# turnDeep/Computational-Chemistry-AI

Measured on AMD Instinct MI355X. Metric: scf_iterations_per_sec, higher is better.
Workload: dtype f64

## Files before the change

computational-chemistry-ai_amd/csrc/mi355scf.hip:

```cpp

#include <hip/hip_runtime.h>
#include <algorithm>
#include <chrono>
#include <cmath>
#include <cstdarg>
#include <cstdint>
#include <cstdio>
#include <cstring>
#include <numeric>
#include <string>
#include <thread>
#include <mutex>
#include <map>
#include <unordered_map>
#include <vector>

#include "../../include/mi355scf.h"
#include "rys_tables.h"

#define LMAX 4
#define LMAX_1E 3
#define NPC ((LMAX + 1) * (LMAX + 2) / 2)
#define BLK 8
#define ATM_SLOTS 6
// ... 329 lines not shown
    double opt_tpq_maxprim = 32.0;
    int opt_eri_tpq = 1;
    int opt_jk_multi_batch = 8;
    int opt_jk_pair = -1;
    int opt_tri_tiles = 1;
    int tri = 1;
    int opt_jk_cache_mb = 160;
    int opt_grad_rows = 1;
    int opt_grad_rows_min = 20;
    int opt_grad_live = 1;
    int opt_jk_kjlt = 0;
    int opt_jk_dpp = 1;
    int opt_jk_pipe = -1;
    int opt_ao_order = 1;
    int opt_ket_cluster = 1;
    int opt_xf_mlds = 0;
    int opt_rys_qpw_maxcomp = 256;
    double opt_rys_qpw_maxprim = 4.0;
    int opt_xf_qpw_max = 40;
    int opt_work_mb = 2048;
    int opt_grad_work_mb = 1024;
    int opt_vmat_fold_mt = 3;
    int opt_rys_fine = 1;
    int opt_eri_fused = 0;
    int opt_task_table = 1;
    int opt_prim_lds = 0;
    int opt_xcd_map = 1;
    int ao_order = 0;
    int *d_perm = nullptr, *d_iperm = nullptr;
    std::vector<int> perm, iperm;
    int opt_vmat_xcd = 1;
    int opt_vmat_wgs = 0;
    int opt_sp2_direct = 0;
    double *d_xt_scratch = nullptr;
};

static inline int pc_index(int la, int lb) { return la * (la + 1) / 2 + lb; }
static inline int ne_of(int la, int lb) { int n = 0; for (int e = la; e <= la + lb; e++) n += ncart(e); return n; }

static double gaussian_int(int n, double a) { return std::tgamma((n + 1) * 0.5) / (2.0 * std::pow(a, (n + 1) * 0.5)); }

static int set_tile_order(mi_ctx *c, int order)
{
    if (c->ao_order == order) return 0;
    const int nbas = c->nbas;
    std::vector<int> seq(nbas);
    std::iota(seq.begin(), seq.end(), 0);
    if (order == 1) std::stable_sort(seq.begin(), seq.end(), [&](int a, int b) { return c->shells[a].l < c->shells[b].l; });
    c->perm.assign(std::max(c->nao, 1), 0);
    c->iperm.assign(std::max(c->nao, 1), 0);
    int pos = 0;
    for (int s_ : seq) {
        ShellH &S = c->shells[s_];
        S.ao = pos;
        for (int m = 0; m < 2 * S.l + 1; m++) { c->perm[S.ao_nat + m] = pos + m; c->iperm[pos + m] = S.ao_nat + m; }
        pos += 2 * S.l + 1;
    }
    HIPCHK(hipMemcpy(c->d_perm, c->perm.data(), sizeof(int) * c->perm.size(), hipMemcpyHostToDevice));
    HIPCHK(hipMemcpy(c->d_iperm, c->iperm.data(), sizeof(int) * c->iperm.size(), hipMemcpyHostToDevice));
    c->ao_order = order;
    return 0;
}

struct HostStash {
    std::mutex mu;
    std::vector<double> h_M, h_prim;
// ... 222 lines not shown
        std::lock_guard<std::mutex> g(H.mu);
        if (c->h_M.capacity() > H.h_M.capacity()) H.h_M.swap(c->h_M);
        if (c->h_prim.capacity() > H.h_prim.capacity()) H.h_prim.swap(c->h_prim);
        if (c->tiles.capacity() > H.tiles.capacity()) H.tiles.swap(c->tiles);
        if (c->tile_off.capacity() > H.tile_off.capacity()) H.tile_off.swap(c->tile_off);
    }
    delete c;
}

extern "C" int mi_ctx_nao(const mi_ctx *c) { return c ? c->nao : -1; }

extern "C" int mi_set_option(mi_ctx *c, const char *key, double value)
{
    if (!c || !key) return fail("mi_set_option: null argument");
    std::string k(key);
    if (k == "runmax") c->opt_runmax = (int)value;
    else if (k == "omega") {
        if (!(value >= 0.0) || !std::isfinite(value)) return fail("mi_set_option: omega must be finite and >= 0");
        c->opt_omega = value;
    }
    else if (k == "jk_waves") c->opt_jk_waves = (int)value;
    else if (k == "jk_nt") c->opt_jk_nt = (int)value;
    else if (k == "jk_pipe") c->opt_jk_pipe = (int)value;
    else if (k == "jk_dpp") c->opt_jk_dpp = (int)value;
    else if (k == "jk_kjlt") c->opt_jk_kjlt = (int)value;
    else if (k == "grad_live") c->opt_grad_live = (int)value;
    else if (k == "grad_rows") c->opt_grad_rows = (int)value;
    else if (k == "grad_rows_min") c->opt_grad_rows_min = (int)value;
    else if (k == "grad_rows_g32") g_rows_g32 = (int)value;
    else if (k == "jk_cache_mb") c->opt_jk_cache_mb = (int)value;
    else if (k == "jk_pair") c->opt_jk_pair = (int)value;
    else if (k == "jk_multi_batch") c->opt_jk_multi_batch = (int)value;
    else if (k == "sp2_direct") c->opt_sp2_direct = (int)value;
    else if (k == "vmat_wgs") c->opt_vmat_wgs = (int)value;
    else if (k == "vmat_xcd") c->opt_vmat_xcd = (int)value;
    else if (k == "tri_tiles") c->opt_tri_tiles = (int)value;
    else if (k == "ao_order") c->opt_ao_order = (int)value;
    else if (k == "ket_cluster") c->opt_ket_cluster = (int)value;
    else if (k == "xcd_map") c->opt_xcd_map = (int)value;
    else if (k == "prim_lds") c->opt_prim_lds = (int)value;
    else if (k == "task_table") c->opt_task_table = (int)value;
    else if (k == "eri_fused") c->opt_eri_fused = (int)value;
    else if (k == "rys_fine") c->opt_rys_fine = (int)value;
    else if (k == "vmat_fold_mt") c->opt_vmat_fold_mt = (int)value;
    else if (k == "work_mb") c->opt_work_mb = (int)value;
    else if (k == "grad_work_mb") c->opt_grad_work_mb = (int)value;
    else if (k == "rys_qpw_maxcomp") c->opt_rys_qpw_maxcomp = (int)value;
    else if (k == "rys_qpw_maxprim") c->opt_rys_qpw_maxprim = value;
    else if (k == "xf_qpw_max") c->opt_xf_qpw_max = (int)value;
    else if (k == "xf_mlds") c->opt_xf_mlds = (int)value;
    else if (k == "eri_tpq") c->opt_eri_tpq = (int)value;
    else if (k == "tpq_maxprim") c->opt_tpq_maxprim = value;
    else if (k == "xf_mfma_min") c->opt_xf_mfma_min = (int)value;
    else if (k == "grad_dtol") c->opt_grad_dtol = value;
    else if (k == "grad_prefetch") c->opt_grad_prefetch = (int)value;
    else return fail("mi_set_option: unknown key '%s'", key);
    return 0;
}

#define NC1 10

__device__ inline void cart_pow(int l, int idx, int &x, int &y, int &z)
{
    int n = 0;
    for (int lx = l; lx >= 0; lx--) {
        int cnt = l - lx + 1;
// ... 6439 lines not shown
    hipLaunchKernelGGL(finalize_fock_kernel, dim3((unsigned)((nn + 255) / 256)), dim3(256), 0, st, c->d_Jacc, with_k ? c->d_Kacc : nullptr,
                       c->ldp, d_h, d_Vun, d_D, kscale, c->nao, d_F, d_part, c->d_perm);
    HIPCHK(hipGetLastError());
    return 0;
}

__global__ __launch_bounds__(256) void commutator_norm_kernel(const double *M, int n, double *E, double *part)
{
    __shared__ double sh[4];
    size_t idx = (size_t)blockIdx.x * blockDim.x + threadIdx.x;
    double s = 0.0;
    if (idx < (size_t)n * n) {
        int r = (int)(idx / n), cidx = (int)(idx - (size_t)r * n);
        double v = M[idx] - M[(size_t)cidx * n + r];
        E[idx] = v;
        s = v * v;
    }
    for (int o = 32; o > 0; o >>= 1) s += __shfl_xor(s, o);
    if ((threadIdx.x & 63) == 0) sh[threadIdx.x >> 6] = s;
    __syncthreads();
    if (threadIdx.x == 0) part[blockIdx.x] = (sh[0] + sh[1]) + (sh[2] + sh[3]);
}

extern "C" int mi_commutator_norm(mi_ctx *c, const double *d_M, double *d_E, double *d_part, void *stream)
{
    if (!c || !d_M || !d_E || !d_part) return fail("mi_commutator_norm: null argument");
    int n = c->nao;
    hipLaunchKernelGGL(commutator_norm_kernel, dim3((unsigned)(((size_t)n * n + 255) / 256)), dim3(256), 0, (hipStream_t)stream, d_M, n, d_E,
                       d_part);
    HIPCHK(hipGetLastError());
    return 0;
}

#define VM_T 64
#define VM_KS 64
#define VM_PAD 2
__global__ __launch_bounds__(256) void xc_vmat_kernel(const double *__restrict__ A, const double *__restrict__ W, int nao, int64_t ng,
                                                      int64_t kchunk, double *C, int xcd_order)
{
    __shared__ double Pa[VM_T][VM_KS + VM_PAD], Pb[VM_T][VM_KS + VM_PAD];
    const int nt = (nao + VM_T - 1) / VM_T, ntt = nt * nt;
    const int L = (int)blockIdx.x;
    int tile, split;
    if (xcd_order) { split = (L & 7) + 8 * (L / (8 * ntt)); tile = (L >> 3) % ntt; }
    else { tile = L % ntt; split = L / ntt; }
    const int m0 = (tile / nt) * VM_T, n0 = (tile % nt) * VM_T;
    const int64_t kbeg = (int64_t)split * kchunk, kend = min(ng, kbeg + kchunk);
    const int wave = threadIdx.x >> 6, lane = threadIdx.x & 63;
    const int qm = (wave >> 1) * 32, qn = (wave & 1) * 32;
    const bool va0 = m0 + qm < nao, va1 = m0 + qm + 16 < nao, vb0 = n0 + qn < nao, vb1 = n0 + qn + 16 < nao;
    d4_t acc[2][2];
#pragma unroll
    for (int a = 0; a < 2; a++)
#pragma unroll
        for (int b = 0; b < 2; b++) acc[a][b] = d4_t{0.0, 0.0, 0.0, 0.0};
    constexpr int PER = VM_T * VM_KS / 256;
    double ra[PER], rb[PER];
    auto gload = [&](int64_t k0) {
#pragma unroll
        for (int u = 0; u < PER; u++) {
            int idx = u * 256 + threadIdx.x;
            int r = idx / VM_KS, k = idx - r * VM_KS;
            int64_t g = k0 + k;
            ra[u] = (m0 + r < nao && g < kend) ? A[(size_t)(m0 + r) * ng + g] : 0.0;
            rb[u] = (n0 + r < nao && g < kend) ? W[(size_t)(n0 + r) * ng + g] : 0.0;
        }
// ... 607 lines not shown
```

computational-chemistry-ai_amd/python/mi355scf/engine.py:

```python
import ctypes
import os

import numpy as np
import torch

_HERE = os.path.dirname(os.path.abspath(__file__))
_CSRC = os.path.normpath(os.path.join(_HERE, "..", "..", "csrc"))
LIB_PATH = os.path.join(_CSRC, "libmi355scf.so")
_lib = None


class EngineError(RuntimeError):
    pass


class EngineOutOfMemory(EngineError):

    def __init__(self, msg, need_bytes, free_bytes):
        super().__init__(msg)
        self.need_bytes, self.free_bytes = need_bytes, free_bytes


MI_ERR_NOMEM = -2

# ... 58 lines not shown
        L.mi_xc_aow.argtypes = [vp, vp, vp, i64, ctypes.c_int, vp, vp]
        L.mi_xc_fxc_prep.argtypes = [ip, dp, dp, ctypes.c_int, vp, vp, i64, ctypes.c_int, ctypes.c_int, vp, vp]
        L.mi_xc_fxc_apply.argtypes = [vp, vp, vp, ctypes.c_int, i64, ctypes.c_int, vp, vp]
        L.mi_xc_eval_mgga.argtypes = [ip, dp, ctypes.c_int, vp, vp, vp, i64, vp, vp, vp]
        L.mi_xc_eval_mgga_spin.argtypes = [ip, dp, ctypes.c_int, vp, vp, vp, vp, vp, i64, vp, vp, vp, vp]
        L.mi_xc_vmat.argtypes = [vp, vp, vp, i64, vp, vp]
        L.mi_xc_vmat_fold.argtypes = [vp, vp, vp, i64, ctypes.c_int, vp, vp]
        L.mi_nystrom_warm.argtypes = [vp, vp, vp, vp, vp, ctypes.c_int, ctypes.c_int, vp]
        L.mi_xc_tail.argtypes = [vp, vp, vp, vp, vp, i64, vp, vp]
        L.mi_build_fock.argtypes = [vp, vp, vp, vp, ctypes.c_int, ctypes.c_double, vp, vp, vp]
        L.mi_nystrom_factor.argtypes = [vp, vp, vp, ctypes.c_int, ctypes.c_int, vp, vp, vp]
        L.mi_sp2_init.argtypes = [vp, vp, vp, vp, vp]
        L.mi_sp2_update.argtypes = [vp, vp, vp, ctypes.c_double, vp, vp]
        L.mi_sp2_iterate.argtypes = [vp, vp, vp, ctypes.c_int, ctypes.c_double, ctypes.c_int, vp, vp, ctypes.POINTER(vp), vp]
        L.mi_sp2_iterate_pingpong.argtypes = [vp, vp, vp, ctypes.c_int, ctypes.c_double, vp, ctypes.POINTER(vp), ctypes.POINTER(vp), vp]
        L.mi_sp2_iterate_planned.argtypes = [vp, vp, vp, vp, ctypes.c_int, dp, ctypes.c_double, vp, ctypes.POINTER(vp), ctypes.POINTER(vp), vp]
        L.mi_grad_1e.argtypes = [vp, vp, vp, vp, vp]
        L.mi_grad_eri.argtypes = [vp, vp, ctypes.c_double, vp, vp]
        L.mi_grad_eri_spin.argtypes = [vp, vp, vp, ctypes.c_double, vp, vp]
        L.mi_grad_eri_sharded.argtypes = [vp, vp, vp, ctypes.c_double, vp, ctypes.c_int, ctypes.c_int, vp]
        L.mi_eri_get_memory.argtypes = [vp, ctypes.POINTER(ctypes.c_int64), ctypes.POINTER(ctypes.c_int64)]
        L.mi_eri_release.argtypes = [vp]
        L.mi_tile_store_allocations.restype = ctypes.c_int64
        L.mi_tile_store_allocations.argtypes = [ctypes.c_int64]
        L.mi_eri_read_quartet.argtypes = [vp, ctypes.c_int, ctypes.c_int, ctypes.c_int, ctypes.c_int, dp]
        L.mi_schwarz_get.argtypes = [vp, dp]
        L.mi_df_build.argtypes = [vp, vp, vp, vp, vp]
        L.mi_df_grad.argtypes = [vp, vp, vp, vp, vp, ctypes.c_int, ctypes.c_int, vp]
        L.mi_reduce_blocks.argtypes = [vp]
        L.mi_plan_shards.argtypes = [ctypes.c_int, dp, ctypes.c_double, ctypes.c_int, ctypes.POINTER(ctypes.c_int64),
                                     ctypes.POINTER(ctypes.c_int64)]
        L.mi_fock_energy.argtypes = [vp, vp, vp, vp, vp, vp, ctypes.c_double, vp, vp, vp]
        L.mi_commutator_norm.argtypes = [vp, vp, vp, vp, vp]
        L.mi_c2s_table.argtypes = [ctypes.c_int, dp]
        L.mi_rys_roots_host.argtypes = [ctypes.c_int, ctypes.c_double, dp, dp]
        L.mi_pcm_pairs.argtypes = [vp, ctypes.c_int, ip]
        L.mi_pcm_eval.argtypes = [vp, vp, ctypes.c_int, vp, ctypes.c_int, i64, vp, vp]
        L.mi_pcm_grad.argtypes = [vp, vp, ctypes.c_int, vp, ctypes.c_int, vp, vp, vp, vp]
        L.mi_pcm_potential.argtypes = [vp, vp, ctypes.c_int, i64, vp, vp, vp, vp, vp]
        L.mi_pcm_fock_chunks.argtypes = [ctypes.c_int, i64]
        L.mi_pcm_fock.argtypes = [vp, vp, ctypes.c_int, i64, vp, ctypes.c_double, ctypes.c_int, vp, vp, vp]
        _lib = L
    return _lib


def plan_shards(nao, qblk, tol, nranks):
    q = np.ascontiguousarray(qblk, dtype=np.float64)
    b = np.zeros(nranks, dtype=np.int64)
    r = np.zeros(nranks, dtype=np.int64)
    i64p = ctypes.POINTER(ctypes.c_int64)
    _check(lib().mi_plan_shards(int(nao), _dp(q), float(tol), int(nranks), b.ctypes.data_as(i64p), r.ctypes.data_as(i64p)))
    return b, r


def tile_store_allocations(min_bytes=0):
    return int(lib().mi_tile_store_allocations(int(min_bytes)))


def release_cache():
    lib().mi_release_cache()


def _check(rc):
    if rc != 0:
        raise EngineError(lib().mi_last_error().decode())

# ... 425 lines not shown
        return (A if res.value == A.data_ptr() else B), (out.value - tr.data_ptr()) // 8

    @property
    def reduce_blocks(self):
        return (self.nao * self.nao + 255) // 256

    def sp2_iterate_planned(self, F, A, B, coef, tr, out_scale=1.0):
        coef = np.ascontiguousarray(coef, dtype=np.float64)
        nit = coef.shape[0] - 1
        out, res = ctypes.c_void_p(), ctypes.c_void_p()
        _check(lib().mi_sp2_iterate_planned(self._h, F.data_ptr(), A.data_ptr(), B.data_ptr(), nit, _dp(coef), float(out_scale),
                                            tr.data_ptr(), ctypes.byref(out), ctypes.byref(res), self._stream()))
        return (A if res.value == A.data_ptr() else B), (out.value - tr.data_ptr()) // 8

    def build_fock(self, D, h, kscale, F, part, with_k=True, vxc_unsym=None):
        if not self.eri_ready:
            self.prepare_eri()
        assert D.is_contiguous() and F.is_contiguous() and part.numel() == self.reduce_blocks and part.is_contiguous()
        assert vxc_unsym is None or vxc_unsym.is_contiguous()
        with torch.cuda.device(self.device):
            _check(lib().mi_build_fock(self._h, D.data_ptr(), h.data_ptr(), vxc_unsym.data_ptr() if vxc_unsym is not None else None,
                                       int(bool(with_k)), float(kscale), F.data_ptr(), part.data_ptr(), self._stream()))
        return F

    def fock_energy(self, h, J, K, Vxc, D, kscale, F, part):
        assert part.numel() == self.reduce_blocks and part.is_contiguous()
        _check(lib().mi_fock_energy(self._h, h.data_ptr(), J.data_ptr(), K.data_ptr() if K is not None else None,
                                    Vxc.data_ptr() if Vxc is not None else None, D.data_ptr(), float(kscale), F.data_ptr(),
                                    part.data_ptr(), self._stream()))

    def commutator_norm(self, M, E, part):
        assert part.numel() == self.reduce_blocks and part.is_contiguous()
        _check(lib().mi_commutator_norm(self._h, M.data_ptr(), E.data_ptr(), part.data_ptr(), self._stream()))

    def diis_errvec(self, sdf, out):
        _check(lib().mi_diis_errvec(self._h, sdf.data_ptr(), out.data_ptr(), self._stream()))

    def diis_combine(self, hist, coef, out):
        c = np.ascontiguousarray(coef, dtype=np.float64)
        _check(lib().mi_diis_combine(self._h, hist.data_ptr(), _dp(c), len(c), out.data_ptr(), self._stream()))

    def diis_dots_dev(self, hist_e, e, n, out):
        _check(lib().mi_diis_dots_dev_n(self._h, hist_e.data_ptr(), e.data_ptr(), n, e.numel(), out.data_ptr(), self._stream()))

    def diis_solve(self, part, m, slot, space, B, coef):
        _check(lib().mi_diis_solve(self._h, part.data_ptr(), m, slot, space, B.data_ptr(), coef.data_ptr(), self._stream()))

    def diis_combine_dev(self, hist, coef, n, out):
        _check(lib().mi_diis_combine_dev_n(self._h, hist.data_ptr(), coef.data_ptr(), n, out.numel(), out.data_ptr(), self._stream()))

    def diis_dots(self, hist_e, e, n):
        out = np.zeros(n)
        _check(lib().mi_diis_dots(self._h, hist_e.data_ptr(), e.data_ptr(), n, _dp(out), self._stream()))
        return out


_WARM = {"started": False}


def _warm_libraries(device, n=32, nocc=24):
    if _WARM["started"] or os.environ.get("MI355_NO_WARMUP"):
        return
    _WARM["started"] = True
    import threading

    def work():
# ... 68 lines not shown
```

computational-chemistry-ai_amd/python/mi355scf/scf.py:

```python
import os
import sys
import time

import numpy as np
import torch

from . import engine as _engine
from .mole import Mole
from .purify import HEAD_MAX, Purifier

AU2DEBYE = 2.541746473

_AUFBAU = [(0, 2), (0, 2), (1, 6), (0, 2), (1, 6), (0, 2), (2, 10), (1, 6)]


def _atom_config(z):
    occ = {}
    left = z
    for l, cap in _AUFBAU:
        if left <= 0:
            break
        n = min(cap, left)
        occ.setdefault(l, []).append(n)
        left -= n
    return occ


class DeviceDIIS:

    MAX_SPACE = 16

    def __init__(self, eng, space=8, nmat=1):
        n = eng.nao
        space = int(space)
        if not 1 <= space <= self.MAX_SPACE:
            raise ValueError(f"diis_space = {space}: the device-side Pulay solve supports 1..{self.MAX_SPACE} vectors")
        self.eng, self.space, self.count = eng, space, 0
        shape = (space, n, n) if nmat == 1 else (space, nmat, n, n)
        self.F = torch.empty(*shape, dtype=torch.float64, device=eng.device)
        self.E = torch.empty(*shape, dtype=torch.float64, device=eng.device)
        self.B = np.zeros((space, space))
        self._e = torch.empty(n, n, dtype=torch.float64, device=eng.device)

    NS = 16

    def _gram_and_solve(self, slot, m):
        if not hasattr(self, "dots_dev"):
            dev = self.F.device
            self.dots_dev = torch.zeros(self.space * self.NS, dtype=torch.float64, device=dev)
            self.B_dev = torch.zeros(self.space, self.space, dtype=torch.float64, device=dev)
            self.coef_dev = torch.zeros(self.space, dtype=torch.float64, device=dev)
        self.eng.diis_dots_dev(self.E, self.E[slot], m, self.dots_dev)
        self.eng.diis_solve(self.dots_dev, m, slot, self.space, self.B_dev, self.coef_dev)
        self._pending = (slot, m)

    def push(self, f, e):
        slot = self.count % self.space
        self.F[slot].copy_(f)
        self.E[slot].copy_(e)
        self.count += 1
        m = min(self.count, self.space)
        self._gram_and_solve(slot, m)
        return m

    def next_slot(self):
        return self.count % self.space

    def push_inplace(self):
        slot = self.count % self.space
        self.count += 1
        m = min(self.count, self.space)
        self._gram_and_solve(slot, m)
        return m

    def extrapolate(self, dots=None):
        _slot, m = self._pending
        out = torch.empty_like(self.F[0])
        self.eng.diis_combine_dev(self.F, self.coef_dev, m, out)
        return out

    def update(self, s, d, f):
        sdf = s @ d @ f
        self.eng.diis_errvec(sdf, self._e)
        slot = self.count % self.space
        self.F[slot].copy_(f)
        self.E[slot].copy_(self._e)
# ... 434 lines not shown
        cache = {}
        sl = mol.aoslice_by_atom()
        for ia in range(mol.natm):
            sym = mol.atom_symbol(ia)
            if mol.atom_charge(ia) == 0:
                continue
            if sym not in cache:
                cache[sym] = _atomic_density(sym, mol.basis, mol.atom_charge(ia))
            p0, p1 = sl[ia, 2], sl[ia, 3]
            dm[p0:p1, p0:p1] = cache[sym]
        return dm

    def _start(self, dm0=None):
        mol = self.mol
        self._setup_once()
        eng = self.engine
        self._purifier.trace_bounds = None
        t0 = time.time()
        if dm0 is None:
            dm0 = self.get_init_guess()
        self.timing["guess_seconds"] = time.time() - t0
        t0 = time.time()
        dm = torch.as_tensor(np.asarray(dm0), dtype=torch.float64, device=eng.device).contiguous()
        if self._nranks > 1:
            from . import parallel
            parallel.broadcast0(dm, self._pg)
        self._fgraph = self._fgraph_seen = None
        st = {"nocc": mol.nelectron // 2, "enuc": mol.energy_nuc(), "cycle": 0, "diis": DeviceDIIS(eng, self.diis_space)}
        st["dmo"] = self._L.T @ dm @ self._L
        self._after_density(st, dm, e_last=None, next_cycle=0)
        self.timing["first_fock_seconds"] = time.time() - t0
        return st

    def _after_density(self, st, dm, e_last, next_cycle, sp2_tr=None, nocc=0, layout=None):
        ctx = self._after_density_launch(st, dm, next_cycle, sp2_tr, layout)
        return self._after_density_finish(st, ctx, e_last, nocc)

    _PIN_DOUBLES = 16384

    def _after_density_launch(self, st, dm, next_cycle, sp2_tr=None, layout=None, projector=False):
        Li = self._Linv
        dm = dm.contiguous()
        self._xc_projector = (dm, st["dmo"], st["nocc"]) if projector else None
        nb = self.engine.reduce_blocks
        self.n_fock_builds = getattr(self, "n_fock_builds", 0) + 1
        head = layout.head if layout is not None and 2 * nb <= HEAD_MAX else None
        if head is not None:
            part = head[HEAD_MAX - 2 * nb:HEAD_MAX]
        else:
            part = torch.empty(2 * nb, dtype=torch.float64, device=dm.device)
        fock, extra = self._fock_energy(dm, part[:nb])
        diis = st["diis"]
        keep = next_cycle >= self.diis_start_cycle
        slot = diis.next_slot()
        fo = torch.matmul(Li @ fock, Li.T, out=diis.F[slot]) if keep else Li @ fock @ Li.T
        m = fo @ st["dmo"]
        eo = diis.E[slot] if keep else torch.empty_like(m)
        self.engine.commutator_norm(m, eo, part[nb:])
        if keep:
            diis.push_inplace()
        if head is not None and extra is None:
            packed = head[HEAD_MAX - 2 * nb:HEAD_MAX + sp2_tr.numel()]
        else:
            parts = [part] + ([extra.reshape(-1)] if extra is not None else []) + ([sp2_tr] if sp2_tr is not None else [])
            packed = torch.cat(parts) if len(parts) > 1 else part
        if self._sync_control_on():
            from . import parallel
            parallel.broadcast0(packed, self._pg)
        ctx = dict(dm=dm, fock=fock, fo=fo, nb=nb, n_extra=0 if extra is None else extra.numel(), has_tr=sp2_tr is not None,
                   layout=layout, lowrank=self._xc_projector is not None,
                   packed=packed, event=None)
        k = packed.numel()
        if k <= self._PIN_DOUBLES:
            pin = getattr(self, "_pin", None)
            if pin is None:
                pin = self._pin = torch.empty(self._PIN_DOUBLES, dtype=torch.float64).pin_memory()
                self._pin_event = torch.cuda.Event()
            pin[:k].copy_(packed, non_blocking=True)
            self._pin_event.record()
            ctx["event"] = self._pin_event
        return ctx

    def _after_density_finish(self, st, ctx, e_last, nocc=0):
        nb = ctx["nb"]
        if ctx["event"] is not None:
            ctx["event"].synchronize()
            vals = self._pin[:ctx["packed"].numel()].numpy().copy()
        else:
            vals = ctx["packed"].cpu().numpy()
        e_el = float(vals[:nb].sum())
        c2 = float(vals[nb:2 * nb].sum())
# ... 41 lines not shown
                return "optimistic", "front_cold", cold_passes
            return None
        if planned_ok and pur.plan is not None:
            return ("planned", "planned_nofront", 0) if settled else ("checked", "checked_unsettled_with_plan", 0)
        if planned_ok and (g > self.sp2_plan_gnorm or not self.sp2_plan_inloop):
            if g > self.sp2_plan_gnorm:
                return ("optimistic", None, cold_passes) if cold_ok else ("checked", None, 0)
            return ("optimistic", "optimistic_noplan", pur.iters) if pur.validated else ("checked", None, 0)
        if planned_ok:
            return "eigh", None, 0
        if sp2 and 0 < nocc < n:
            return ("optimistic", None, pur.iters) if pur.validated else ("checked", None, 0)
        return "eigh", None, 0

    def _purify(self, route, fo, nocc, passes):
        pur = self._purifier
        if route == "planned":
            return pur.planned(fo, nocc)
        if route == "optimistic":
            return pur.optimistic(fo, nocc, passes)
        return pur.checked(fo, nocc), None, None

    def _front(self, st):
        r = self._route(st, head=True)
        if r is None:
            return None
        route, label, passes = r
        if route == "planned" and self.graph_front:
            out = self._front_graphed(st, st["nocc"])
            if out is not None:
                return out
        fo = st["diis"].extrapolate()
        dmo, tr_dev, layout = self._purify(route, fo, st["nocc"], passes)
        dm = (self._Linv.T @ dmo @ self._Linv).contiguous()
        return dict(fo=fo, dmo=dmo, dm=dm, tr=tr_dev, layout=layout, route=route, label=label)

    graph_front = True
    _GRAPH_STABLE = 3

    def _front_graphed(self, st, nocc):
        diis = st["diis"]
        pur = self._purifier
        m = min(diis.count, diis.space)
        key = (id(diis), m, pur.plan_len, pur.plan_gen, self._Linv.data_ptr())
        g = self.__dict__.get("_fgraph")
        if g is None or g["key"] != key or g["diis"] is not diis:
            seen = self.__dict__.get("_fgraph_seen")
            if seen is None or seen[0] != key:
                self._fgraph_seen = [key, 1]
                return None
            seen[1] += 1
            if seen[1] < self._GRAPH_STABLE or m < diis.space:
                return None
            g = self._fgraph = dict(key=key, diis=diis, heads=[], turn=0)
        i, g["turn"] = g["turn"], 1 - g["turn"]
        if i < len(g["heads"]):
            head = g["heads"][i]
            head["graph"].replay()
            return head["out"]
        try:
            def body():
                fo = diis.extrapolate()
                dmo, tr_dev, layout = pur.planned(fo, nocc, slot=1 - i)
                dm = torch.matmul(self._Linv.T @ dmo, self._Linv)
                return dict(fo=fo, dmo=dmo, dm=dm, tr=tr_dev, layout=layout, route="planned", label="front_planned")
            cur = torch.cuda.current_stream()
            side = torch.cuda.Stream()
            side.wait_stream(cur)
            with torch.cuda.stream(side):
                body()
            cur.wait_stream(side)
            graph = torch.cuda.CUDAGraph()
            with torch.cuda.graph(graph):
                out = body()
            graph.replay()
            g["heads"].append(dict(graph=graph, out=out))
            return out
        except Exception as e:
            self.graph_front = False
            self._fgraph = None
            self._log(4, f"HIP-graph capture of the SCF head failed ({e!r}); continuing with eager launches")
            return None

    def _step(self, st, use_diis=True, want_mo=False):
        nocc, Li = st["nocc"], self._Linv
        pur = self._purifier
        front = st.pop("front", None)
        if want_mo or not use_diis:
            front = None
        paths = self.__dict__.setdefault("path_counts", {})

        def took(name):
            paths[name] = paths.get(name, 0) + 1

        def eigh(fo):
            e, c = torch.linalg.eigh(fo)
            co = c[:, :nocc]
            return e, c, 2.0 * co @ co.T
        if front is not None:
            fo, dmo, tr_dev, layout, dm, route = (front[k] for k in ("fo", "dmo", "tr", "layout", "dm", "route"))
            took(front["label"])
            st.pop("mo_e", None)
        else:
            if use_diis and st["cycle"] >= self.diis_start_cycle:
                fo = st["diis"].extrapolate()
            else:
                fo = st["fo"]
            if self.level_shift and use_diis:
                fo = fo + self.level_shift * (torch.eye(fo.shape[0], dtype=fo.dtype, device=fo.device) - 0.5 * st["dmo"])
            route, label, passes = self._route(st, want_mo=want_mo)
            if label:
                took(label)
            dmo, tr_dev, layout = (None, None, None) if route == "eigh" else self._purify(route, fo, nocc, passes)
            if dmo is None:
                took("eigh")
                e, c, dmo = eigh(fo)
                st.update(mo_e=e, mo_c=Li.T @ c)
                if self.eig_method == "sp2" and not self.level_shift and (want_mo or (self.sp2_planned and 0 < nocc < fo.shape[0])):
                    pur.replan(e, nocc)
            else:
                st.pop("mo_e", None)
            dm = Li.T @ dmo @ Li
        saved = (st["dmo"], st["diis"].count)
        st["dmo"] = dmo
        e_prev = st["e_tot"]
        ctx = self._after_density_launch(st, dm, st["cycle"] + 1, sp2_tr=tr_dev, layout=layout, projector=True)
        nxt = self._front(st) if (use_diis and not want_mo) else None
        if (self.sp2_trace_plan and pur.plan is None and pur.trace_bounds is not None and use_diis and not want_mo
                and st.get("gnorm", 1.0) <= self.sp2_trace_plan_gnorm):
            if pur.plan_from_traces():
                took("plan_from_traces")
        ok = self._after_density_finish(st, ctx, e_prev, nocc)
        if not ok:
            nxt = None
            self.n_redo = getattr(self, "n_redo", 0) + 1
            st["dmo"], st["diis"].count = saved
            st["e_tot"] = e_prev
            pur.validated = False
            redo, _, _ = self._route(st, redo_of=route)
            dmo = pur.checked(fo, nocc) if redo == "checked" else None
            if dmo is None:
                e, _c, dmo = eigh(fo)
                if redo == "eigh":
                    pur.replan(e, nocc)
            st["dmo"] = dmo
            self._after_density(st, Li.T @ dmo @ Li, e_last=e_prev, next_cycle=st["cycle"] + 1)
        if nxt is not None:
            st["front"] = nxt
        st["cycle"] += 1
        return st

    def kernel(self, dm0=None, **kw):
        t_start = time.time()
        st = self._start(dm0)
        eng = self.engine
        conv_tol = self.conv_tol
        conv_tol_grad = self.conv_tol_grad if self.conv_tol_grad is not None else np.sqrt(conv_tol)
        self._log(4, f"init E= {st['e_tot']:.15g}")
        self.converged = False
        t_loop = time.time()
        while st["cycle"] < self.max_cycle:
            self._step(st)
            self._log(4, f"cycle= {st['cycle']} E= {st['e_tot']:.15g}  delta_E= {st['de']:.3g}  |g|= {st['gnorm']:.3g}")
            if abs(st["de"]) < conv_tol and st["gnorm"] < conv_tol_grad:
                self.converged = True
                break
        st.pop("front", None)
        self.cycles = st["cycle"]
        self.timing["loop_seconds"] = time.time() - t_loop
        t_final = time.time()
        if self.converged and self.conv_check:
            self._step(st, use_diis=False, want_mo=True)
            self._log(4, f"Extra cycle  E= {st['e_tot']:.15g}  delta_E= {st['de']:.3g}")
        if "mo_e" not in st:
            e_, c_ = torch.linalg.eigh(st["fo"])
            st["mo_e"], st["mo_c"] = e_, self._Linv.T @ c_
            if self.eig_method == "sp2" and not self.level_shift:
                self._purifier.replan(e_, st["nocc"])
        self._dm, self._vhf = st["dm"], st["fock"] - self._h1
# ... 144 lines not shown
```

include/mi355scf.h:

```cpp
#ifndef MI355SCF_H
#define MI355SCF_H

#include <stddef.h>
#include <stdint.h>

#ifdef __cplusplus
extern "C" {
#endif

typedef struct mi_ctx mi_ctx;

const char *mi_last_error(void);

int mi_abi_version(void);

int mi_ctx_create(const int32_t *atm, int natm, const int32_t *bas, int nbas, const double *env,
                  int nenv, int device_id, mi_ctx **out);
void mi_ctx_destroy(mi_ctx *ctx);
int mi_ctx_nao(const mi_ctx *ctx);

void mi_release_cache(void);

int mi_set_option(mi_ctx *ctx, const char *key, double value);

// ... 36 lines not shown
int mi_time_jk_variant(mi_ctx *ctx, const double *d_D, int with_j, int with_k, int reps, double *ms_per_launch,
                       void *stream);

int mi_diis_errvec(mi_ctx *ctx, const double *d_SDF, double *d_err, void *stream);
int mi_diis_combine(mi_ctx *ctx, const double *d_hist, const double *coef, int n, double *d_out,
                    void *stream);
int mi_diis_dots(mi_ctx *ctx, const double *d_hist_e, const double *d_e, int n, double *out,
                 void *stream);
int mi_diis_dots_dev(mi_ctx *ctx, const double *d_hist_e, const double *d_e, int n, double *d_out,
                     void *stream);
int mi_diis_solve(mi_ctx *ctx, const double *d_part, int m, int slot, int space, double *d_B, double *d_coef, void *stream);
int mi_diis_combine_dev(mi_ctx *ctx, const double *d_hist, const double *d_coef, int n, double *d_out, void *stream);
int mi_diis_dots_dev_n(mi_ctx *ctx, const double *d_hist_e, const double *d_e, int n, int64_t len, double *d_out, void *stream);
int mi_diis_combine_dev_n(mi_ctx *ctx, const double *d_hist, const double *d_coef, int n, int64_t len, double *d_out, void *stream);


int mi_sp2_init(mi_ctx *ctx, const double *d_F, double *d_X, double *d_work, void *stream);
int mi_sp2_update(mi_ctx *ctx, double *d_X, const double *d_X2, double n_occ, double *d_out_with_traces,
                  void *stream);

int mi_sp2_iterate(mi_ctx *ctx, double *d_X, double *d_X2, int nit, double n_occ, int have_x2,
                   double *d_work, double *d_tr, double **d_tr_out, void *stream);
int mi_sp2_iterate_pingpong(mi_ctx *ctx, double *d_A, double *d_B, int nit, double n_occ, double *d_tr, double **d_tr_out,
                            double **d_res, void *stream);

int mi_sp2_iterate_planned(mi_ctx *ctx, const double *d_F, double *d_A, double *d_B, int nit, const double *coef, double out_scale,
                           double *d_tr, double **d_tr_out, double **d_res, void *stream);

int mi_reduce_blocks(const mi_ctx *ctx);
int mi_fock_energy(mi_ctx *ctx, const double *d_h, const double *d_J, const double *d_K, const double *d_Vxc,
                   const double *d_D, double kscale, double *d_F, double *d_part, void *stream);
int mi_commutator_norm(mi_ctx *ctx, const double *d_M, double *d_E, double *d_part, void *stream);


int mi_grid_becke(mi_ctx *ctx, const double *d_coords, const int32_t *d_atom_of, const double *d_vol,
                  int64_t ng, const double *d_adjust, double *d_weights, void *stream);

int mi_eval_ao(mi_ctx *ctx, const double *d_coords, int64_t ng, int deriv, double *d_ao, void *stream);

int mi_xc_rho(mi_ctx *ctx, const double *d_ao, const double *d_C, int64_t ng, int deriv, double *d_rho,
              void *stream);
int mi_xc_rho_mo(mi_ctx *ctx, const double *d_psi, int nocc, int64_t ng, int deriv, double *d_rho, double *d_tau, void *stream);
int mi_build_fock(mi_ctx *ctx, const double *d_D, const double *d_h, const double *d_Vun, int with_k, double kscale, double *d_F,
                  double *d_part, void *stream);
int mi_nystrom_warm(mi_ctx *ctx, const double *d_Zt, const int *d_info, const double *d_G0, double *d_G, int nocc, int n,
                    void *stream);
int mi_nystrom_factor(mi_ctx *ctx, const double *d_M, const double *d_W, int n, int nocc, double *d_Zt, int *d_info, void *stream);
int mi_xc_tail(mi_ctx *ctx, const double *d_w, const double *d_v0, const double *d_v1, const double *d_v2, int64_t ng, double *d_tail,
               void *stream);
int mi_xc_rho_lowrank(mi_ctx *ctx, const double *d_ao, const double *d_Zp, int ldz, int64_t ng, int deriv, double *d_rho,
                      double *d_tau, void *stream);

int mi_xc_eval(const int32_t *kinds, const double *coefs, int nterms, const double *d_rho,
               const double *d_w, int64_t ng, int gga, double *d_exc, double *d_wv, double *d_vrho,
               double *d_vsigma, void *stream);
int mi_xc_eval_spin(const int32_t *kinds, const double *coefs, int nterms, const double *d_rhoa, const double *d_rhob,
                    const double *d_w, int64_t ng, int gga, double *d_exc, double *d_wva, double *d_wvb, void *stream);
int mi_xc_eval_p(const int32_t *kinds, const double *coefs, const double *params, int nterms, const double *d_rho,
                 const double *d_w, int64_t ng, int gga, double *d_exc, double *d_wv, double *d_vrho, double *d_vsigma, void *stream);
int mi_xc_eval_spin_p(const int32_t *kinds, const double *coefs, const double *params, int nterms, const double *d_rhoa,
                      const double *d_rhob, const double *d_w, int64_t ng, int gga, double *d_exc, double *d_wva, double *d_wvb,
                      void *stream);

int mi_xc_fxc_prep(const int32_t *kinds, const double *coefs, const double *params, int nterms, const double *d_rho,
                   const double *d_w, int64_t ng, int gga, int triplet, double *d_coef, void *stream);
int mi_xc_fxc_apply(const double *d_rho0, const double *d_coef, const double *d_rho1, int m, int64_t ng, int gga, double *d_wv1,
// ... 40 lines not shown
```

Before: 967.2.

## Fuse SCF tail: triangular congruence, fused commutator norm, single-launch DIIS push

Adds MFMA-based kernels for the per-iteration SCF tail. The orthogonal-basis transforms Li·F·Liᵀ and Liᵀ·D·Li use the triangular structure of Linv and write only symmetric halves. The commutator FD−DF and its norm are computed in one kernel without a separate matmul. The DIIS dot products and the small linear solve run in one launch, with a last-block ticket. This cuts kernel launches and skips the zero half of the triangular factor, at the cost of custom code limited to small nao and atomic ticket synchronization.

After: 1026, median of 6. 1.06x the previous value.

```diff
diff --git a/computational-chemistry-ai_amd/csrc/mi355scf.hip b/computational-chemistry-ai_amd/csrc/mi355scf.hip
--- a/computational-chemistry-ai_amd/csrc/mi355scf.hip
+++ b/computational-chemistry-ai_amd/csrc/mi355scf.hip
@@ -385,6 +385,7 @@
     int opt_vmat_xcd = 1;
     int opt_vmat_wgs = 0;
     int opt_sp2_direct = 0;
+    int opt_tail_fused = 1;
     double *d_xt_scratch = nullptr;
 };
 
@@ -673,6 +674,7 @@
     else if (k == "jk_pair") c->opt_jk_pair = (int)value;
     else if (k == "jk_multi_batch") c->opt_jk_multi_batch = (int)value;
     else if (k == "sp2_direct") c->opt_sp2_direct = (int)value;
+    else if (k == "tail_fused") c->opt_tail_fused = (int)value;
     else if (k == "vmat_wgs") c->opt_vmat_wgs = (int)value;
     else if (k == "vmat_xcd") c->opt_vmat_xcd = (int)value;
     else if (k == "tri_tiles") c->opt_tri_tiles = (int)value;
@@ -7178,6 +7180,289 @@
     return 0;
 }
 
+template <int MS>
+__device__ __forceinline__ d4_t ptq_partial(const double *P, const double *Q, int n, int i0, int j0, int klo, int Sb)
+{
+    const int wave = (threadIdx.x >> 6) & 3, lane = threadIdx.x & 63, col = lane & 15, g = lane >> 4;
+    const int ia = i0 + col, jb = j0 + col, ca = min(ia, n - 1), cb = min(jb, n - 1);
+    const int kw = klo + wave * 4 * Sb + g;
+    const int kend = min(klo + 16 * Sb, n);
+    double a[MS], b[MS];
+#pragma unroll
+    for (int s = 0; s < MS; s++) {
+        const size_t row = (size_t)min(kw + 4 * s, kend - 1) * n;
+        a[s] = P[row + ca];
+        b[s] = Q[row + cb];
+    }
+#pragma unroll
+    for (int s = 0; s < MS; s++) {
+        const bool in = s < Sb && kw + 4 * s < kend;
+        a[s] = (in && ia < n) ? a[s] : 0.0;
+        b[s] = (in && jb < n) ? b[s] : 0.0;
+    }
+    d4_t acc0 = {0.0, 0.0, 0.0, 0.0}, acc1 = {0.0, 0.0, 0.0, 0.0};
+#pragma unroll
+    for (int s = 0; s < MS; s += 2) {
+        if (s < Sb) acc0 = __builtin_amdgcn_mfma_f64_16x16x4f64(a[s], b[s], acc0, 0, 0, 0);
+        if (s + 1 < MS && s + 1 < Sb) acc1 = __builtin_amdgcn_mfma_f64_16x16x4f64(a[s + 1], b[s + 1], acc1, 0, 0, 0);
+    }
+    d4_t r;
+#pragma unroll
+    for (int q = 0; q < 4; q++) r[q] = acc0[q] + acc1[q];
+    return r;
+}
+__device__ __forceinline__ d4_t ptq_partial_any(const double *P, const double *Q, int n, int i0, int j0, int klo, int Sb)
+{
+    if (Sb <= 4) return ptq_partial<4>(P, Q, n, i0, j0, klo, Sb);
+    if (Sb <= 8) return ptq_partial<8>(P, Q, n, i0, j0, klo, Sb);
+    if (Sb <= 12) return ptq_partial<12>(P, Q, n, i0, j0, klo, Sb);
+    if (Sb <= 16) return ptq_partial<16>(P, Q, n, i0, j0, klo, Sb);
+    return ptq_partial<SP2_DIRECT_MAXS>(P, Q, n, i0, j0, klo, Sb);
+}
+__device__ __forceinline__ void ptq_stage(const d4_t &acc, double *red)
+{
+    const int wave = (threadIdx.x >> 6) & 3, lane = threadIdx.x & 63;
+#pragma unroll
+    for (int q = 0; q < 4; q++) red[wave * 256 + q * 64 + lane] = acc[q];
+}
+__device__ __forceinline__ double ptq_sum4(const double *red, int e)
+{
+    return (red[e] + red[256 + e]) + (red[512 + e] + red[768 + e]);
+}
+
+template <bool TRI>
+__global__ __launch_bounds__(256) void congruence_kernel(const double *P, const double *Q, int n, int lower, double *out)
+{
+    __shared__ double red[4 * 256];
+    const int T = (n + 15) >> 4;
+    int bI, bJ;
+    if (TRI) sp2_tile_of_block((int)blockIdx.x, bI, bJ);
+    else { bI = (int)blockIdx.x / T; bJ = (int)blockIdx.x - bI * T; }
+    const int bt = TRI ? bI : bJ;
+    const int klo = lower ? 16 * bt : 0, Sb = lower ? T - bt : bt + 1;
+    const int i0 = 16 * bI, j0 = 16 * bJ;
+    ptq_stage(ptq_partial_any(P, Q, n, i0, j0, klo, Sb), red);
+    __syncthreads();
+    const int e = threadIdx.x, gi = i0 + (e >> 4), gj = j0 + (e & 15);
+    if (gi < n && gj < n && (!TRI || gi >= gj)) {
+        const double v = ptq_sum4(red, e);
+        out[(size_t)gi * n + gj] = v;
+        if (TRI && gi != gj) out[(size_t)gj * n + gi] = v;
+    }
+}
+
+static int tail_fused_ok(const mi_ctx *c) { return c->opt_tail_fused && (c->nao + 15) / 16 <= SP2_DIRECT_MAXS; }
+
+extern "C" int mi_tail_fused(const mi_ctx *c) { return c ? tail_fused_ok(c) : 0; }
+
+extern "C" int mi_congruence(mi_ctx *c, const double *d_At, int lower, const double *d_X, double *d_T, double *d_Y, void *stream)
+{
+    if (!c || !d_At || !d_X || !d_T || !d_Y) return fail("mi_congruence: null argument");
+    if (d_T == d_X || d_T == d_Y || d_T == d_At || d_Y == d_At) return fail("mi_congruence: the scratch and the result must not alias an operand");
+    const int n = c->nao, T = (n + 15) / 16;
+    if (T > SP2_DIRECT_MAXS) return fail("mi_congruence: nao = %d is above the register-operand limit %d", n, 16 * SP2_DIRECT_MAXS);
+    hipStream_t st = (hipStream_t)stream;
+    hipLaunchKernelGGL(congruence_kernel<false>, dim3((unsigned)(T * T)), dim3(256), 0, st, d_X, d_At, n, lower != 0, d_T);
+    hipLaunchKernelGGL(congruence_kernel<true>, dim3((unsigned)(T * (T + 1) / 2)), dim3(256), 0, st, d_At, (const double *)d_T, n, lower != 0, d_Y);
+    HIPCHK(hipGetLastError());
+    return 0;
+}
+
+__global__ __launch_bounds__(512) void commutator_fused_kernel(const double *F, const double *D, int n, double *E, double *part, int npart)
+{
+    __shared__ double red[2][4 * 256];
+    __shared__ double sh[4];
+    const int T = (n + 15) >> 4, npairs = T * (T + 1) / 2;
+    const int half = threadIdx.x >> 8, e = threadIdx.x & 255;
+    double s = 0.0;
+    for (int p = (int)blockIdx.x; p < npairs; p += (int)gridDim.x) {
+        int bI, bJ;
+        sp2_tile_of_block(p, bI, bJ);
+        const bool diag = bI == bJ;
+        const int i0 = 16 * bI, j0 = 16 * bJ;
+        if (half == 0) ptq_stage(ptq_partial_any(F, D, n, i0, j0, 0, T), red[0]);
+        else if (!diag) ptq_stage(ptq_partial_any(F, D, n, j0, i0, 0, T), red[1]);
+        __syncthreads();
+        if (half == 0) {
+            const int r = e >> 4, cc = e & 15, gi = i0 + r, gj = j0 + cc;
+            if (gi < n && gj < n) {
+                const double v = ptq_sum4(red[0], e) - ptq_sum4(red[diag ? 0 : 1], cc * 16 + r);
+                E[(size_t)gi * n + gj] = v;
+                if (!diag) E[(size_t)gj * n + gi] = -v;
+                s += diag ? v * v : 2.0 * (v * v);
+            }
+        }
+        __syncthreads();
+    }
+    if (half == 0) {
+        for (int o = 32; o > 0; o >>= 1) s += __shfl_xor(s, o);
+        if ((e & 63) == 0) sh[e >> 6] = s;
+    }
+    __syncthreads();
+    if (threadIdx.x == 0) part[blockIdx.x] = (sh[0] + sh[1]) + (sh[2] + sh[3]);
+    if (blockIdx.x == 0)
+        for (int i = (int)gridDim.x + (int)threadIdx.x; i < npart; i += (int)blockDim.x) part[i] = 0.0;
+}
+
+extern "C" int mi_commutator_fused(mi_ctx *c, const double *d_F, const double *d_D, double *d_E, double *d_part, void *stream)
+{
+    if (!c || !d_F || !d_D || !d_E || !d_part) return fail("mi_commutator_fused: null argument");
+    if (d_E == d_F || d_E == d_D) return fail("mi_commutator_fused: the result must not alias an operand");
+    const int n = c->nao, T = (n + 15) / 16, nb = (int)(((size_t)n * n + 255) / 256);
+    if (T > SP2_DIRECT_MAXS) return fail("mi_commutator_fused: nao = %d is above the register-operand limit %d", n, 16 * SP2_DIRECT_MAXS);
+    const int grid = std::min(T * (T + 1) / 2, nb);
+    hipLaunchKernelGGL(commutator_fused_kernel, dim3((unsigned)grid), dim3(512), 0, (hipStream_t)stream, d_F, d_D, n, d_E, d_part, nb);
+    HIPCHK(hipGetLastError());
+    return 0;
+}
+
+__device__ void diis_solve_block(const double *part, int m, int slot, int space, double *B, double *coef, double *lds)
+{
+    constexpr int NR = DIIS_MAXM + 1, LD = DIIS_MAXM + 3;
+    double *A = lds, *X = lds + NR * LD;
+    const int t = threadIdx.x, n = m + 1, w = n + 1;
+    int er[2], ej[2];
+    double bold[2];
+#pragma unroll
+    for (int u = 0; u < 2; u++) {
+        const int el = t + 256 * u;
+        er[u] = el / w;
+        ej[u] = el - er[u] * w;
+        if (er[u] >= n) er[u] = -1;
+        const bool gram = er[u] >= 1 && ej[u] >= 1 && ej[u] < n && er[u] - 1 != slot && ej[u] - 1 != slot;
+        bold[u] = gram ? B[(er[u] - 1) * space + ej[u] - 1] : 0.0;
+    }
+    if (t < m) {
+        double pq[DIIS_NS], dot = 0.0;
+#pragma unroll
+        for (int q = 0; q < DIIS_NS; q++) pq[q] = part[t * DIIS_NS + q];
+#pragma unroll
+        for (int q = 0; q < DIIS_NS; q++) dot += pq[q];
+        B[slot * space + t] = dot;
+        B[t * space + slot] = dot;
+        X[t] = dot;
+    }
+    __syncthreads();
+#pragma unroll
+    for (int u = 0; u < 2; u++) {
+        const int r = er[u], j = ej[u];
+        if (r < 0) continue;
+        const double xj = X[min(max(j - 1, 0), DIIS_MAXM - 1)], xr = X[max(r - 1, 0)];
+        double v;
+        if (j == n) v = (r == 0) ? 1.0 : 0.0;
+        else if (r == 0) v = (j == 0) ? 0.0 : 1.0;
+        else if (j == 0) v = 1.0;
+        else if (r - 1 == slot) v = xj;
+        else if (j - 1 == slot) v = xr;
+        else v = bold[u];
+        A[r * LD + j] = v;
+    }
+    __syncthreads();
+    bool ok = true;
+    for (int k = 0; k < n; k++) {
+        double cv[NR];
+        int ci[NR];
+#pragma unroll
+        for (int r = 0; r < NR; r++) {
+            cv[r] = fabs(A[r * LD + k]);
+            ci[r] = r;
+        }
+#pragma unroll
+        for (int r = 0; r < NR; r++) cv[r] = (r >= k && r < n) ? cv[r] : -1.0;
+#pragma unroll
+        for (int st = 1; st < NR; st <<= 1)
+#pragma unroll
+            for (int i = 0; i + st < NR; i += 2 * st)
+                if (cv[i + st] > cv[i]) { cv[i] = cv[i + st]; ci[i] = ci[i + st]; }
+        const double val = cv[0];
+        const int p = ci[0];
+        if (!(val > 0.0) || !isfinite(val)) { ok = false; break; }
+        double nv[2];
+#pragma unroll
+        for (int u = 0; u < 2; u++) {
+            const int r = max(er[u], 0), j = ej[u];
+            const int src = (r == p) ? k : r;
+            const double piv = A[p * LD + j], num = A[src * LD + k], den = A[p * LD + k], own = A[src * LD + j];
+            nv[u] = (r == k) ? piv : fma(-(num / den), piv, own);
+        }
+        __syncthreads();
+#pragma unroll
+        for (int u = 0; u < 2; u++)
+            if (er[u] >= k && ej[u] >= k) A[er[u] * LD + ej[u]] = nv[u];
+        __syncthreads();
+    }
+    if (t >= 64) return;
+    double U[NR], rhs = 0.0, x = 0.0;
+#pragma unroll
+    for (int j = 0; j < NR; j++) U[j] = A[min(t, NR - 1) * LD + j];
+#pragma unroll
+    for (int j = 0; j < NR; j++) U[j] = (t < n && j < n) ? U[j] : 1.0;
+    if (t < n) rhs = A[t * LD + n];
+    if (ok) {
+#pragma unroll
+        for (int i = NR - 1; i >= 0; i--) {
+            if (i < n) {
+                const double xi = lane_bcast(rhs / U[i], i);
+                if (!isfinite(xi)) ok = false;
+                if (t < i) rhs = fma(-U[i], xi, rhs);
+                if (t == i) x = xi;
+            }
+        }
+    }
+    if (t >= 1 && t <= m) coef[t - 1] = ok ? x : ((t - 1) == slot ? 1.0 : 0.0);
+}
+
+__global__ __launch_bounds__(256) void diis_dots_solve_kernel(const double *hist, const double *e, size_t nn, double *part, int slot, int space,
+                                                              double *B, double *coef, unsigned *ticket)
+{
+    __shared__ double lds[(DIIS_MAXM + 1) * (DIIS_MAXM + 3) + DIIS_MAXM + 8];
+    double *sh = lds;
+    const double *h = hist + (size_t)blockIdx.x * nn;
+    const size_t per = (nn + DIIS_NS - 1) / DIIS_NS, lo = per * blockIdx.y, hi = lo + per < nn ? lo + per : nn;
+    double p[4] = {0, 0, 0, 0};
+    size_t i = lo + threadIdx.x;
+    for (; i + 3 * 256 < hi; i += 4 * 256) {
+#pragma unroll
+        for (int u = 0; u < 4; u++) p[u] = fma(h[i + u * 256], e[i + u * 256], p[u]);
+    }
+    for (; i < hi; i += 256) p[0] = fma(h[i], e[i], p[0]);
+    double s = (p[0] + p[1]) + (p[2] + p[3]);
+    for (int o = 32; o > 0; o >>= 1) s += __shfl_xor(s, o);
+    if ((threadIdx.x & 63) == 0) sh[threadIdx.x >> 6] = s;
+    __syncthreads();
+    if (threadIdx.x == 0) part[blockIdx.x * DIIS_NS + blockIdx.y] = (sh[0] + sh[1]) + (sh[2] + sh[3]);
+    asm volatile("s_waitcnt vmcnt(0)" ::: "memory");
+    __syncthreads();
+    if (threadIdx.x == 0) {
+        __builtin_amdgcn_fence(__ATOMIC_RELEASE, "agent");
+        asm volatile("s_waitcnt vmcnt(0)" ::: "memory");
+        const unsigned total = gridDim.x * gridDim.y;
+        const bool last = __hip_atomic_fetch_add(ticket, 1u, __ATOMIC_RELAXED, __HIP_MEMORY_SCOPE_AGENT) == total - 1;
+        if (last) {
+            __hip_atomic_store(ticket, 0u, __ATOMIC_RELAXED, __HIP_MEMORY_SCOPE_AGENT);
+            __builtin_amdgcn_fence(__ATOMIC_ACQUIRE, "agent");
+            asm volatile("s_waitcnt vmcnt(0)" ::: "memory");
+        }
+        sh[4] = last ? 1.0 : 0.0;
+    }
+    __syncthreads();
+    if (sh[4] == 0.0) return;
+    __syncthreads();
+    diis_solve_block(part, (int)gridDim.x, slot, space, B, coef, lds);
+}
+
+extern "C" int mi_diis_push(mi_ctx *c, const double *d_hist_e, const double *d_e, int m, int slot, int space, int64_t len, double *d_part,
+                            double *d_B, double *d_coef, void *d_ticket, void *stream)
+{
+    if (!c || !d_hist_e || !d_e || !d_part || !d_B || !d_coef || !d_ticket || len < 1 || m < 1 || m > DIIS_MAXM || space < m || slot < 0 ||
+        slot >= m)
+        return fail("mi_diis_push: bad argument");
+    hipLaunchKernelGGL(diis_dots_solve_kernel, dim3(m, DIIS_NS), dim3(256), 0, (hipStream_t)stream, d_hist_e, d_e, (size_t)len, d_part, slot, space,
+                       d_B, d_coef, (unsigned *)d_ticket);
+    HIPCHK(hipGetLastError());
+    return 0;
+}
+
 #define VM_T 64
 #define VM_KS 64
 #define VM_PAD 2
diff --git a/computational-chemistry-ai_amd/python/mi355scf/engine.py b/computational-chemistry-ai_amd/python/mi355scf/engine.py
--- a/computational-chemistry-ai_amd/python/mi355scf/engine.py
+++ b/computational-chemistry-ai_amd/python/mi355scf/engine.py
@@ -114,6 +114,10 @@
                                      ctypes.POINTER(ctypes.c_int64)]
         L.mi_fock_energy.argtypes = [vp, vp, vp, vp, vp, vp, ctypes.c_double, vp, vp, vp]
         L.mi_commutator_norm.argtypes = [vp, vp, vp, vp, vp]
+        L.mi_tail_fused.argtypes = [vp]
+        L.mi_congruence.argtypes = [vp, vp, ctypes.c_int, vp, vp, vp, vp]
+        L.mi_commutator_fused.argtypes = [vp, vp, vp, vp, vp, vp]
+        L.mi_diis_push.argtypes = [vp, vp, vp, ctypes.c_int, ctypes.c_int, ctypes.c_int, ctypes.c_int64, vp, vp, vp, vp, vp]
         L.mi_c2s_table.argtypes = [ctypes.c_int, dp]
         L.mi_rys_roots_host.argtypes = [ctypes.c_int, ctypes.c_double, dp, dp]
         L.mi_pcm_pairs.argtypes = [vp, ctypes.c_int, ip]
@@ -605,6 +609,30 @@
     def commutator_norm(self, M, E, part):
         assert part.numel() == self.reduce_blocks and part.is_contiguous()
         _check(lib().mi_commutator_norm(self._h, M.data_ptr(), E.data_ptr(), part.data_ptr(), self._stream()))
+
+    @property
+    def tail_fused(self):
+        want = int(os.environ.get("MI355_TAIL_FUSED", "1") != "0")
+        if getattr(self, "_tail_fused_set", None) != want:
+            self.set_option("tail_fused", want)
+            self._tail_fused_set = want
+        return bool(lib().mi_tail_fused(self._h))
+
+    def congruence(self, At, lower, X, out=None):
+        assert At.is_contiguous() and X.is_contiguous() and (out is None or out.is_contiguous())
+        out = torch.empty_like(X) if out is None else out
+        scratch = torch.empty_like(X)
+        _check(lib().mi_congruence(self._h, At.data_ptr(), int(bool(lower)), X.data_ptr(), scratch.data_ptr(),
+                                   out.data_ptr(), self._stream()))
+        return out
+
+    def commutator_fused(self, F, D, E, part):
+        assert part.numel() == self.reduce_blocks and part.is_contiguous() and F.is_contiguous() and D.is_contiguous() and E.is_contiguous()
+        _check(lib().mi_commutator_fused(self._h, F.data_ptr(), D.data_ptr(), E.data_ptr(), part.data_ptr(), self._stream()))
+
+    def diis_push(self, hist_e, e, m, slot, space, part, B, coef, ticket):
+        _check(lib().mi_diis_push(self._h, hist_e.data_ptr(), e.data_ptr(), m, slot, space, e.numel(), part.data_ptr(), B.data_ptr(),
+                                  coef.data_ptr(), ticket.data_ptr(), self._stream()))
 
     def diis_errvec(self, sdf, out):
         _check(lib().mi_diis_errvec(self._h, sdf.data_ptr(), out.data_ptr(), self._stream()))
diff --git a/computational-chemistry-ai_amd/python/mi355scf/scf.py b/computational-chemistry-ai_amd/python/mi355scf/scf.py
--- a/computational-chemistry-ai_amd/python/mi355scf/scf.py
+++ b/computational-chemistry-ai_amd/python/mi355scf/scf.py
@@ -50,8 +50,12 @@
             self.dots_dev = torch.zeros(self.space * self.NS, dtype=torch.float64, device=dev)
             self.B_dev = torch.zeros(self.space, self.space, dtype=torch.float64, device=dev)
             self.coef_dev = torch.zeros(self.space, dtype=torch.float64, device=dev)
-        self.eng.diis_dots_dev(self.E, self.E[slot], m, self.dots_dev)
-        self.eng.diis_solve(self.dots_dev, m, slot, self.space, self.B_dev, self.coef_dev)
+            self.ticket = torch.zeros(4, dtype=torch.int32, device=dev)
+        if self.eng.tail_fused:
+            self.eng.diis_push(self.E, self.E[slot], m, slot, self.space, self.dots_dev, self.B_dev, self.coef_dev, self.ticket)
+        else:
+            self.eng.diis_dots_dev(self.E, self.E[slot], m, self.dots_dev)
+            self.eng.diis_solve(self.dots_dev, m, slot, self.space, self.B_dev, self.coef_dev)
         self._pending = (slot, m)
 
     def push(self, f, e):
@@ -552,6 +556,28 @@
         self.timing["first_fock_seconds"] = time.time() - t0
         return st
 
+    def _tri(self):
+        if not self.engine.tail_fused:
+            return None
+        t = self.__dict__.get("_tri_ops")
+        if t is None or t[0] != self._Linv.data_ptr():
+            li = torch.tril(self._Linv).contiguous()
+            t = self._tri_ops = (self._Linv.data_ptr(), li, li.T.contiguous())
+        return t[1], t[2]
+
+    def _fock_orth(self, fock, out=None):
+        tri = self._tri()
+        if tri is not None:
+            return self.engine.congruence(tri[1], False, fock, out=out)
+        Li = self._Linv
+        return Li @ fock @ Li.T if out is None else torch.matmul(Li @ fock, Li.T, out=out)
+
+    def _density_ao(self, dmo):
+        tri = self._tri()
+        if tri is not None:
+            return self.engine.congruence(tri[0], True, dmo.contiguous())
+        return torch.matmul(self._Linv.T @ dmo, self._Linv)
+
     def _after_density(self, st, dm, e_last, next_cycle, sp2_tr=None, nocc=0, layout=None):
         ctx = self._after_density_launch(st, dm, next_cycle, sp2_tr, layout)
         return self._after_density_finish(st, ctx, e_last, nocc)
@@ -559,7 +585,6 @@
     _PIN_DOUBLES = 16384
 
     def _after_density_launch(self, st, dm, next_cycle, sp2_tr=None, layout=None, projector=False):
-        Li = self._Linv
         dm = dm.contiguous()
         self._xc_projector = (dm, st["dmo"], st["nocc"]) if projector else None
         nb = self.engine.reduce_blocks
@@ -573,10 +598,12 @@
         diis = st["diis"]
         keep = next_cycle >= self.diis_start_cycle
         slot = diis.next_slot()
-        fo = torch.matmul(Li @ fock, Li.T, out=diis.F[slot]) if keep else Li @ fock @ Li.T
-        m = fo @ st["dmo"]
-        eo = diis.E[slot] if keep else torch.empty_like(m)
-        self.engine.commutator_norm(m, eo, part[nb:])
+        fo = self._fock_orth(fock, out=diis.F[slot] if keep else None)
+        eo = diis.E[slot] if keep else torch.empty_like(fo)
+        if self.engine.tail_fused:
+            self.engine.commutator_fused(fo, st["dmo"].contiguous(), eo, part[nb:])
+        else:
+            self.engine.commutator_norm(fo @ st["dmo"], eo, part[nb:])
         if keep:
             diis.push_inplace()
         if head is not None and extra is None:
@@ -684,7 +711,7 @@
                 return out
         fo = st["diis"].extrapolate()
         dmo, tr_dev, layout = self._purify(route, fo, st["nocc"], passes)
-        dm = (self._Linv.T @ dmo @ self._Linv).contiguous()
+        dm = self._density_ao(dmo)
         return dict(fo=fo, dmo=dmo, dm=dm, tr=tr_dev, layout=layout, route=route, label=label)
 
     graph_front = True
@@ -714,7 +741,7 @@
             def body():
                 fo = diis.extrapolate()
                 dmo, tr_dev, layout = pur.planned(fo, nocc, slot=1 - i)
-                dm = torch.matmul(self._Linv.T @ dmo, self._Linv)
+                dm = self._density_ao(dmo)
                 return dict(fo=fo, dmo=dmo, dm=dm, tr=tr_dev, layout=layout, route="planned", label="front_planned")
             cur = torch.cuda.current_stream()
             side = torch.cuda.Stream()
@@ -772,7 +799,7 @@
                     pur.replan(e, nocc)
             else:
                 st.pop("mo_e", None)
-            dm = Li.T @ dmo @ Li
+            dm = self._density_ao(dmo)
         saved = (st["dmo"], st["diis"].count)
         st["dmo"] = dmo
         e_prev = st["e_tot"]
@@ -796,7 +823,7 @@
                 if redo == "eigh":
                     pur.replan(e, nocc)
             st["dmo"] = dmo
-            self._after_density(st, Li.T @ dmo @ Li, e_last=e_prev, next_cycle=st["cycle"] + 1)
+            self._after_density(st, self._density_ao(dmo), e_last=e_prev, next_cycle=st["cycle"] + 1)
         if nxt is not None:
             st["front"] = nxt
         st["cycle"] += 1
diff --git a/include/mi355scf.h b/include/mi355scf.h
--- a/include/mi355scf.h
+++ b/include/mi355scf.h
@@ -92,6 +92,12 @@
                    const double *d_D, double kscale, double *d_F, double *d_part, void *stream);
 int mi_commutator_norm(mi_ctx *ctx, const double *d_M, double *d_E, double *d_part, void *stream);
 
+int mi_tail_fused(const mi_ctx *ctx);
+int mi_congruence(mi_ctx *ctx, const double *d_At, int lower, const double *d_X, double *d_T, double *d_Y, void *stream);
+int mi_commutator_fused(mi_ctx *ctx, const double *d_F, const double *d_D, double *d_E, double *d_part, void *stream);
+int mi_diis_push(mi_ctx *ctx, const double *d_hist_e, const double *d_e, int m, int slot, int space, int64_t len, double *d_part,
+                 double *d_B, double *d_coef, void *d_ticket, void *stream);
+
 
 int mi_grid_becke(mi_ctx *ctx, const double *d_coords, const int32_t *d_atom_of, const double *d_vol,
                   int64_t ng, const double *d_adjust, double *d_weights, void *stream);
```
